# alguoo314/JASPER

Measured on AMD Instinct MI355X. Metric: assembly Mbp/s polished + Gk-mers/s counted, k=37, higher is better.
Workload: dtype u64

## Files before the change

include/jasper_hip.h:

```cpp
#ifndef JASPER_HIP_H
#define JASPER_HIP_H
#include <stddef.h>
#include <stdint.h>

#ifdef __cplusplus
extern "C" {
#endif

typedef struct jasper_table jasper_table;
typedef struct jasper_result jasper_result;

typedef struct jasper_fixrec {
    int64_t index;
    uint32_t chunk;
    uint32_t seqno;
    uint8_t pass;
    uint8_t kind;
    uint8_t newc;
    uint8_t oldc;
    uint32_t rep;
    uint32_t aux_off;
    uint32_t aux_len;
} jasper_fixrec;

#define JASPER_OK 0
#define JASPER_ERR -1
#define JASPER_ERR_CAPACITY -2
#define JASPER_ERR_FORMAT -3
#define JASPER_ERR_REFERENCE_EXIT -4

const char *jasper_last_error(void);
int jasper_device_count(int *n);
int jasper_request_cancel(int on);
int jasper_device_mem_info(int device, uint64_t *free_bytes, uint64_t *total_bytes);

int jasper_table_create(int k, uint64_t min_slots, int device, jasper_table **out);
int jasper_table_load_jf(const char *path, int device, jasper_table **out);
void jasper_table_destroy(jasper_table *t);
int jasper_table_load_jf_part(const char *path, int device, uint32_t part, uint32_t nparts, jasper_table **out);
int jasper_table_write_jf(jasper_table *t, const char *path, const char *const *cmdline, int n_cmdline);
int jasper_debug_mix(int k, int inverse, uint64_t hi, uint64_t lo, uint64_t out2[2]);
int jasper_table_info(jasper_table *t, int *k, uint64_t *slots, uint64_t *distinct, uint64_t *occurrences);
int jasper_table_sync(jasper_table *t);
int jasper_table_clear(jasper_table *t);

int jasper_count_bases(jasper_table *t, const char *bases, uint64_t n);
int jasper_count_bases_device(jasper_table *t, const void *d_bases, uint64_t n);
int jasper_count_reads_text(jasper_table *t, const char *text, uint64_t n);
int jasper_count_reads_files(jasper_table *t, const char *const *paths, int n_paths);
int jasper_count_reads_file_ranges(jasper_table *t, const char *const *paths, const int64_t *begins, const int64_t *ends, int n_paths);

int jasper_last_ingest(jasper_table *t, uint64_t *gpu_bytes, uint64_t *host_bytes);
int jasper_last_inflate(jasper_table *t, uint64_t stats[6]);
int jasper_histogram(jasper_table *t, uint64_t *out10002);
int jasper_histogram_part(jasper_table *t, uint32_t part, uint32_t nparts, uint64_t *out10002);
int jasper_histogram_is_fused(jasper_table *t);
int jasper_lookup(jasper_table *t, const char *chars, const int64_t *offsets, uint64_t n, uint32_t *out);

int jasper_table_export(jasper_table *t, uint64_t *n_entries, uint64_t *host_entries );
int jasper_table_import(jasper_table *t, const uint64_t *host_entries, uint64_t n_entries);
int jasper_table_export_device(jasper_table *t, uint64_t *n_entries, void **d_entries);
int jasper_table_import_device(jasper_table *t, const void *d_entries, uint64_t n_entries);
int jasper_table_export_to(jasper_table *t, void *d_dst, uint64_t cap_entries, uint64_t *n_entries);
int jasper_device_free(jasper_table *t, void *d_ptr);
int jasper_table_export_packed(jasper_table *t, void *d_dst, uint64_t cap_entries, uint64_t *n_entries, uint32_t part, uint32_t nparts);
int jasper_table_import_packed(jasper_table *t, const void *d_src, uint64_t n_entries, int mode);
int jasper_table_import_packed_multi(jasper_table *t, const void *const *d_srcs, const uint64_t *counts, uint32_t n_src);
int jasper_table_reserve(jasper_table *t, uint64_t min_slots);
int jasper_table_fit(jasper_table *t, double max_load);

int jasper_table_export_owner(jasper_table *t, void *d_dst, uint64_t cap_entries, uint32_t n_owners, uint64_t *counts);
int jasper_read_feed_start(jasper_table *t, const char *const *paths, const int64_t *begins, const int64_t *ends, int n_paths);
int jasper_read_feed_next(jasper_table *t, const void **d_bases, uint64_t *n);
int jasper_read_feed_release(jasper_table *t);
int jasper_count_exchange_plan(jasper_table *t, uint64_t piece_max, uint64_t records_max, uint32_t n_owners, uint64_t *out8);
int jasper_count_exchange_scan(jasper_table *t, const void *d_bases, uint64_t n, uint64_t pos, uint64_t end, uint64_t piece_max, uint32_t n_owners, void *d_deferred,
                               uint64_t deferred_cap, uint64_t *records);
int jasper_count_exchange_partition(jasper_table *t, uint64_t piece_max, uint64_t records_max, uint32_t n_owners, void *d_send, void *d_send_counts, void *d_deferred,
                                    uint64_t deferred_cap);
int jasper_count_exchange_dedupe(jasper_table *t, uint64_t piece_max, uint64_t records_max, uint32_t n_owners, void *d_send, void *d_send_counts, uint32_t *max_fill,
                                 int *count_bits);
int jasper_count_exchange_insert(jasper_table *t, const void *d_recv, const void *d_recv_counts, uint64_t piece_max, uint64_t records_max, uint32_t n_owners,
                                 uint32_t self, const void *d_deferred_all, uint64_t n_deferred_all, int whole_input, uint32_t slice_cap, int count_bits);
int jasper_table_export_file_ranges(jasper_table *t, void *d_dst, uint64_t cap_entries, uint32_t n_ranges, int size_log2, uint64_t *counts);
int jasper_table_write_jf_piece(jasper_table *t, const char *path, const char *const *cmdline, int n_cmdline, int size_log2, int what);
int jasper_table_ipc_handle(jasper_table *t, void *out64);
int jasper_table_attach_ipc(jasper_table *t, const void *handles, uint32_t n, uint32_t self);
int jasper_table_attach_tables(jasper_table *t, jasper_table *const *shards, uint32_t n, uint32_t self);
int jasper_table_detach(jasper_table *t);
int jasper_ipc_probe(int device, const void *handles, uint32_t n, uint32_t self);
uint32_t jasper_owner_of(uint64_t hash_lo, uint64_t hash_hi, uint32_t n);

int jasper_polish_batch(jasper_table *t, int n_chunks, const char *const *seqs, const int64_t *lens,
                        int solid_thre, int passes, int fix, jasper_result **out);
int jasper_polish_batch_device(jasper_table *t, int n_chunks, const void *d_text, const int64_t *offsets,
                               int solid_thre, int passes, int fix, jasper_result **out);
int jasper_result_num_chunks(const jasper_result *r);
int jasper_result_seq(const jasper_result *r, int chunk, const char **seq, int64_t *len);
int jasper_result_seq_len(const jasper_result *r, int chunk, int64_t *len);
int jasper_result_seq_device(const jasper_result *r, int chunk, const void **d_seq, int64_t *len);
int jasper_result_records(const jasper_result *r, const jasper_fixrec **recs, uint64_t *n);
int jasper_result_aux(const jasper_result *r, int chunk, const char **aux, uint64_t *n);
int jasper_result_qv(const jasper_result *r, int64_t out4[4]);
int jasper_result_qv_chunk(const jasper_result *r, int chunk, int64_t out4[4]);
int jasper_result_lookups(const jasper_result *r, uint64_t *n);
double jasper_result_seconds(const jasper_result *r);
int jasper_result_segments(const jasper_result *r, uint64_t *n_segments, uint64_t *n_respeculated);
int jasper_polish_cut_geometry(int k, int64_t out5[5]);
int jasper_result_retried(const jasper_result *r);
void jasper_result_free(jasper_result *r);

typedef struct jasper_report jasper_report;
typedef struct jasper_kmer_run { int64_t start; uint64_t n_kmers; uint64_t n_absent; uint32_t seq; uint32_t min_count; } jasper_kmer_run;
int jasper_kmer_report(jasper_table *t, int n_seqs, const char *const *seqs, const int64_t *lens, uint32_t thre, jasper_report **out);
int jasper_kmer_report_device(jasper_table *t, int n_seqs, const void *d_text, const int64_t *offsets, uint32_t thre, jasper_report **out);
int jasper_report_tile_windows(void);
int jasper_report_num_seqs(const jasper_report *r);
int jasper_report_counts(const jasper_report *r, int seq, uint64_t out4[4]);
int jasper_report_runs(const jasper_report *r, const jasper_kmer_run **runs, uint64_t *n);
double jasper_report_seconds(const jasper_report *r);
int jasper_report_retried(const jasper_report *r);
void jasper_report_free(jasper_report *r);

int jasper_spectrum_rows(void);
int jasper_table_spectrum(jasper_table *reads, jasper_table *assembly, uint64_t *out_cells , double *device_seconds);
// ... 227 lines not shown
```

jasper_amd/_lib.py:

```python
import ctypes as C
import os

_HERE = os.path.dirname(os.path.abspath(__file__))
LIB_PATH = os.environ.get("JASPER_AMD_LIB") or os.path.join(_HERE, "libjasper_hip.so")

JASPER_OK = 0
JASPER_ERR = -1
JASPER_ERR_CAPACITY = -2
JASPER_ERR_FORMAT = -3
JASPER_ERR_REFERENCE_EXIT = -4


class FixRec(C.Structure):
    _fields_ = [("index", C.c_int64), ("chunk", C.c_uint32), ("seqno", C.c_uint32), ("pass_", C.c_uint8),
                ("kind", C.c_uint8), ("newc", C.c_uint8), ("oldc", C.c_uint8), ("rep", C.c_uint32),
                ("aux_off", C.c_uint32), ("aux_len", C.c_uint32)]


assert C.sizeof(FixRec) == 32


class KmerRun(C.Structure):
    _fields_ = [("start", C.c_int64), ("n_kmers", C.c_uint64), ("n_absent", C.c_uint64), ("seq", C.c_uint32), ("min_count", C.c_uint32)]

# ... 22 lines not shown

assert C.sizeof(HapRun) == 24


class Variant(C.Structure):
    _fields_ = [("pos", C.c_int64), ("seq", C.c_uint32), ("ref_min", C.c_uint32), ("alt_min", C.c_uint32), ("ref", C.c_uint8), ("alt", C.c_uint8),
                ("kind", C.c_uint8), ("pad", C.c_uint8)]


assert C.sizeof(Variant) == 24


class Indel(C.Structure):
    _fields_ = [("pos", C.c_int64), ("seq", C.c_uint32), ("ref_min", C.c_uint32), ("alt_min", C.c_uint32), ("len", C.c_uint16), ("type", C.c_uint8),
                ("base", C.c_uint8), ("kind", C.c_uint8), ("pad", C.c_uint8 * 7)]


assert C.sizeof(Indel) == 32


class MixedIns(C.Structure):
    _fields_ = [("pos", C.c_int64), ("seq", C.c_uint32), ("ref_min", C.c_uint32), ("alt_min", C.c_uint32), ("bases", C.c_uint32), ("len", C.c_uint16),
                ("kind", C.c_uint8), ("pad", C.c_uint8 * 5)]


assert C.sizeof(MixedIns) == 32


class Compound(C.Structure):
    _fields_ = [("pos", C.c_int64), ("seq", C.c_uint32), ("ref_min", C.c_uint32), ("alt_min", C.c_uint32), ("ref_len", C.c_uint32), ("bases", C.c_uint64 * 2),
                ("len", C.c_uint16), ("pad", C.c_uint8 * 6)]


assert C.sizeof(Compound) == 48


class HetCluster(C.Structure):
    _fields_ = Compound._fields_


assert C.sizeof(HetCluster) == 48


class Edit(C.Structure):
    _fields_ = [("pos", C.c_int64), ("seq", C.c_uint32), ("ref_min", C.c_uint32), ("alt_min", C.c_uint32), ("ref_len", C.c_uint32), ("bases", C.c_uint64 * 2),
                ("len", C.c_uint16), ("source", C.c_uint8), ("round", C.c_uint8), ("pad", C.c_uint8 * 4)]


assert C.sizeof(Edit) == 48


class RepairRound(C.Structure):
    _fields_ = [("records", C.c_uint64), ("accepted", C.c_uint64), ("conflicts", C.c_uint64), ("ambiguous", C.c_uint64), ("unreliable_before", C.c_uint64),
                ("unreliable_after", C.c_uint64)]


assert C.sizeof(RepairRound) == 48


class GapSite(C.Structure):
    _fields_ = [("a", C.c_int64), ("q", C.c_int64), ("seq", C.c_uint32), ("ref_min", C.c_uint32), ("n_records", C.c_uint32), ("levels", C.c_uint32),
                ("trim_left", C.c_uint32), ("trim_right", C.c_uint32), ("kind", C.c_uint8), ("status", C.c_uint8), ("pad", C.c_uint8 * 6)]


assert C.sizeof(GapSite) == 48


class GapFill(C.Structure):
    _fields_ = [("pos", C.c_int64), ("bases_off", C.c_uint64), ("seq", C.c_uint32), ("ref_len", C.c_uint32), ("len", C.c_uint32), ("alt_min", C.c_uint32)]


assert C.sizeof(GapFill) == 32

_P = C.c_void_p
SYMBOLS = {
    "jasper_last_error": (C.c_char_p, []),
    "jasper_device_count": (C.c_int, [C.POINTER(C.c_int)]),
    "jasper_request_cancel": (C.c_int, [C.c_int]),
    "jasper_device_mem_info": (C.c_int, [C.c_int, C.POINTER(C.c_uint64), C.POINTER(C.c_uint64)]),
    "jasper_table_create": (C.c_int, [C.c_int, C.c_uint64, C.c_int, C.POINTER(_P)]),
    "jasper_table_load_jf": (C.c_int, [C.c_char_p, C.c_int, C.POINTER(_P)]),
    "jasper_table_destroy": (None, [_P]),
    "jasper_table_info": (C.c_int, [_P, C.POINTER(C.c_int), C.POINTER(C.c_uint64), C.POINTER(C.c_uint64), C.POINTER(C.c_uint64)]),
    "jasper_table_sync": (C.c_int, [_P]),
    "jasper_table_clear": (C.c_int, [_P]),
    "jasper_count_bases": (C.c_int, [_P, C.c_char_p, C.c_uint64]),
    "jasper_count_bases_device": (C.c_int, [_P, _P, C.c_uint64]),
    "jasper_count_reads_text": (C.c_int, [_P, C.c_char_p, C.c_uint64]),
    "jasper_count_reads_files": (C.c_int, [_P, C.POINTER(C.c_char_p), C.c_int]),
    "jasper_count_reads_file_ranges": (C.c_int, [_P, C.POINTER(C.c_char_p), C.POINTER(C.c_int64), C.POINTER(C.c_int64), C.c_int]),
    "jasper_table_load_jf_part": (C.c_int, [C.c_char_p, C.c_int, C.c_uint32, C.c_uint32, C.POINTER(_P)]),
    "jasper_table_write_jf": (C.c_int, [_P, C.c_char_p, C.POINTER(C.c_char_p), C.c_int]),
    "jasper_debug_mix": (C.c_int, [C.c_int, C.c_int, C.c_uint64, C.c_uint64, C.POINTER(C.c_uint64)]),
    "jasper_last_ingest": (C.c_int, [_P, C.POINTER(C.c_uint64), C.POINTER(C.c_uint64)]),
    "jasper_last_inflate": (C.c_int, [_P, C.POINTER(C.c_uint64)]),
    "jasper_histogram_part": (C.c_int, [_P, C.c_uint32, C.c_uint32, C.POINTER(C.c_uint64)]),
    "jasper_histogram_is_fused": (C.c_int, [_P]),
    "jasper_histogram": (C.c_int, [_P, C.POINTER(C.c_uint64)]),
    "jasper_lookup": (C.c_int, [_P, C.c_char_p, C.POINTER(C.c_int64), C.c_uint64, C.POINTER(C.c_uint32)]),
    "jasper_table_export": (C.c_int, [_P, C.POINTER(C.c_uint64), C.POINTER(C.c_uint64)]),
    "jasper_table_import": (C.c_int, [_P, C.POINTER(C.c_uint64), C.c_uint64]),
    "jasper_table_export_device": (C.c_int, [_P, C.POINTER(C.c_uint64), C.POINTER(_P)]),
    "jasper_table_import_device": (C.c_int, [_P, _P, C.c_uint64]),
    "jasper_table_export_to": (C.c_int, [_P, _P, C.c_uint64, C.POINTER(C.c_uint64)]),
    "jasper_device_free": (C.c_int, [_P, _P]),
    "jasper_table_export_packed": (C.c_int, [_P, _P, C.c_uint64, C.POINTER(C.c_uint64), C.c_uint32, C.c_uint32]),
    "jasper_table_import_packed": (C.c_int, [_P, _P, C.c_uint64, C.c_int]),
    "jasper_table_import_packed_multi": (C.c_int, [_P, C.POINTER(_P), C.POINTER(C.c_uint64), C.c_uint32]),
    "jasper_table_reserve": (C.c_int, [_P, C.c_uint64]),
    "jasper_table_fit": (C.c_int, [_P, C.c_double]),
    "jasper_read_feed_start": (C.c_int, [_P, C.POINTER(C.c_char_p), C.POINTER(C.c_int64), C.POINTER(C.c_int64), C.c_int]),
    "jasper_read_feed_next": (C.c_int, [_P, C.POINTER(C.c_void_p), C.POINTER(C.c_uint64)]),
    "jasper_read_feed_release": (C.c_int, [_P]),
    "jasper_count_exchange_plan": (C.c_int, [_P, C.c_uint64, C.c_uint64, C.c_uint32, C.POINTER(C.c_uint64)]),
    "jasper_count_exchange_scan": (C.c_int, [_P, _P, C.c_uint64, C.c_uint64, C.c_uint64, C.c_uint64, C.c_uint32, _P, C.c_uint64, C.POINTER(C.c_uint64)]),
    "jasper_count_exchange_partition": (C.c_int, [_P, C.c_uint64, C.c_uint64, C.c_uint32, _P, _P, _P, C.c_uint64]),
    "jasper_count_exchange_dedupe": (C.c_int, [_P, C.c_uint64, C.c_uint64, C.c_uint32, _P, _P, C.POINTER(C.c_uint32), C.POINTER(C.c_int)]),
    "jasper_count_exchange_insert": (C.c_int, [_P, _P, _P, C.c_uint64, C.c_uint64, C.c_uint32, C.c_uint32, _P, C.c_uint64, C.c_int, C.c_uint32, C.c_int]),
    "jasper_table_export_owner": (C.c_int, [_P, _P, C.c_uint64, C.c_uint32, C.POINTER(C.c_uint64)]),
    "jasper_table_export_file_ranges": (C.c_int, [_P, _P, C.c_uint64, C.c_uint32, C.c_int, C.POINTER(C.c_uint64)]),
    "jasper_table_write_jf_piece": (C.c_int, [_P, C.c_char_p, C.POINTER(C.c_char_p), C.c_int, C.c_int, C.c_int]),
    "jasper_table_ipc_handle": (C.c_int, [_P, _P]),
    "jasper_table_attach_ipc": (C.c_int, [_P, _P, C.c_uint32, C.c_uint32]),
    "jasper_table_attach_tables": (C.c_int, [_P, C.POINTER(_P), C.c_uint32, C.c_uint32]),
    "jasper_table_detach": (C.c_int, [_P]),
    "jasper_ipc_probe": (C.c_int, [C.c_int, _P, C.c_uint32, C.c_uint32]),
    "jasper_table_release_retired": (C.c_int, [_P]),
    "jasper_inflate_file": (C.c_int, [C.c_char_p, C.c_int, C.c_uint64, C.c_char_p, C.POINTER(C.c_uint64), C.POINTER(C.c_int)]),
    "jasper_inflate_file_device": (C.c_int, [C.c_int, C.c_char_p, C.c_uint64, C.c_char_p, C.POINTER(C.c_uint64), C.POINTER(C.c_uint64)]),
    "jasper_owner_of": (C.c_uint32, [C.c_uint64, C.c_uint64, C.c_uint32]),
    "jasper_polish_batch": (C.c_int, [_P, C.c_int, C.POINTER(C.c_char_p), C.POINTER(C.c_int64), C.c_int, C.c_int, C.c_int, C.POINTER(_P)]),
    "jasper_result_num_chunks": (C.c_int, [_P]),
    "jasper_polish_batch_device": (C.c_int, [_P, C.c_int, _P, C.POINTER(C.c_int64), C.c_int, C.c_int, C.c_int, C.POINTER(_P)]),
    "jasper_result_seq": (C.c_int, [_P, C.c_int, C.POINTER(_P), C.POINTER(C.c_int64)]),
    "jasper_result_seq_len": (C.c_int, [_P, C.c_int, C.POINTER(C.c_int64)]),
    "jasper_result_seq_device": (C.c_int, [_P, C.c_int, C.POINTER(_P), C.POINTER(C.c_int64)]),
    "jasper_result_records": (C.c_int, [_P, C.POINTER(C.POINTER(FixRec)), C.POINTER(C.c_uint64)]),
    "jasper_result_aux": (C.c_int, [_P, C.c_int, C.POINTER(_P), C.POINTER(C.c_uint64)]),
    "jasper_result_qv": (C.c_int, [_P, C.POINTER(C.c_int64)]),
    "jasper_result_qv_chunk": (C.c_int, [_P, C.c_int, C.POINTER(C.c_int64)]),
    "jasper_result_lookups": (C.c_int, [_P, C.POINTER(C.c_uint64)]),
    "jasper_result_seconds": (C.c_double, [_P]),
    "jasper_result_segments": (C.c_int, [_P, C.POINTER(C.c_uint64), C.POINTER(C.c_uint64)]),
    "jasper_polish_cut_geometry": (C.c_int, [C.c_int, C.POINTER(C.c_int64)]),
    "jasper_result_retried": (C.c_int, [_P]),
    "jasper_result_free": (None, [_P]),
    "jasper_kmer_report": (C.c_int, [_P, C.c_int, C.POINTER(C.c_char_p), C.POINTER(C.c_int64), C.c_uint32, C.POINTER(_P)]),
    "jasper_kmer_report_device": (C.c_int, [_P, C.c_int, _P, C.POINTER(C.c_int64), C.c_uint32, C.POINTER(_P)]),
    "jasper_report_tile_windows": (C.c_int, []),
    "jasper_report_num_seqs": (C.c_int, [_P]),
    "jasper_report_counts": (C.c_int, [_P, C.c_int, C.POINTER(C.c_uint64)]),
    "jasper_report_runs": (C.c_int, [_P, C.POINTER(C.POINTER(KmerRun)), C.POINTER(C.c_uint64)]),
    "jasper_report_seconds": (C.c_double, [_P]),
    "jasper_report_retried": (C.c_int, [_P]),
    "jasper_report_free": (None, [_P]),
    "jasper_spectrum_rows": (C.c_int, []),
    "jasper_table_spectrum": (C.c_int, [_P, _P, C.POINTER(C.c_uint64), C.POINTER(C.c_double)]),
    "jasper_copy_report": (C.c_int, [_P, _P, C.c_int, C.POINTER(C.c_char_p), C.POINTER(C.c_int64), C.c_uint32, C.c_uint32, C.POINTER(_P)]),
    "jasper_copy_report_device": (C.c_int, [_P, _P, C.c_int, _P, C.POINTER(C.c_int64), C.c_uint32, C.c_uint32, C.POINTER(_P)]),
    "jasper_copyrep_num_seqs": (C.c_int, [_P]),
    "jasper_copyrep_counts": (C.c_int, [_P, C.c_int, C.POINTER(C.c_uint64)]),
    "jasper_copyrep_runs": (C.c_int, [_P, C.POINTER(C.POINTER(CopyRun)), C.POINTER(C.c_uint64)]),
    "jasper_copyrep_seconds": (C.c_double, [_P]),
    "jasper_copyrep_retried": (C.c_int, [_P]),
    "jasper_copyrep_free": (None, [_P]),
    "jasper_dup_map": (C.c_int, [_P, _P, C.c_int, C.POINTER(C.c_char_p), C.POINTER(C.c_int64), C.c_uint32, C.c_uint32, C.POINTER(_P)]),
# ... 174 lines not shown
```

jasper_amd/csrc/capi.hip:

```cpp
#include "../../include/jasper_hip.h"
#include "ingest.hpp"
#include "polish_host.hpp"
#include "table.hpp"
#include "pgunzip.hpp"
#include "inflate_gpu.hpp"
#include "asmio.hpp"
#include "report.hpp"
#include "spectra.hpp"
#include "copies.hpp"
#include "hapmers.hpp"
#include "variants.hpp"
#include "indels.hpp"
#include "compound.hpp"
#include "repair.hpp"
#include "dups.hpp"
#include "gaps.hpp"
#include <zlib.h>
#include <algorithm>
#include <cmath>
#include <cstddef>
#include <cstring>
#include <string>
#include <vector>

// ... 134 lines not shown

int jasper_request_cancel(int on) { jk::g_cancel.store(on ? 1 : 0); return JASPER_OK; }

int jasper_device_mem_info(int device, uint64_t *free_bytes, uint64_t *total_bytes) {
    size_t f = 0, t = 0;
    hipError_t e = hipSetDevice(device);
    if (e == hipSuccess) e = hipMemGetInfo(&f, &t);
    if (e != hipSuccess) { g_err = std::string("hipMemGetInfo: ") + hipGetErrorString(e); return JASPER_ERR; }
    if (free_bytes) *free_bytes = (uint64_t)f;
    if (total_bytes) *total_bytes = (uint64_t)t;
    return JASPER_OK;
}

int jasper_table_create(int k, uint64_t min_slots, int device, jasper_table **out) {
    if (!out) { g_err = "null out"; return JASPER_ERR; }
    jasper_table *h = new jasper_table();
    int rc = h->t.init(k, min_slots, device, g_err);
    if (rc) { h->t.destroy(); delete h; return rc; }
    *out = h;
    return JASPER_OK;
}

int jasper_table_load_jf(const char *path, int device, jasper_table **out) {
    if (!out || !path) { g_err = "null argument"; return JASPER_ERR; }
    JfHeader h;
    int rc = jf_read_header(path, h, g_err);
    if (rc) return rc == -3 ? JASPER_ERR_FORMAT : JASPER_ERR;
    jasper_table *t = nullptr;
    rc = jasper_table_create(h.key_len / 2, std::max<uint64_t>(1u << 16, 2 * h.n_records), device, &t);
    if (rc) return rc;
    Table *T = &t->t;
    rc = T->load_jf_records(path, h.data_offset, h.n_records, h.key_len, h.counter_len, g_err);
    if (rc) { jasper_table_destroy(t); return rc < -1 ? rc : JASPER_ERR; }
    *out = t;
    return JASPER_OK;
}

int jasper_table_load_jf_part(const char *path, int device, uint32_t part, uint32_t nparts, jasper_table **out) {
    if (!out || !path || nparts == 0 || part >= nparts) { g_err = "bad argument"; return JASPER_ERR; }
    JfHeader h;
    int rc = jf_read_header(path, h, g_err);
    if (rc) return rc == -3 ? JASPER_ERR_FORMAT : JASPER_ERR;
    const uint64_t lo = h.n_records / nparts * part + std::min<uint64_t>(part, h.n_records % nparts);
    const uint64_t n = h.n_records / nparts + (part < h.n_records % nparts ? 1 : 0);
    const uint64_t rec = (uint64_t)((h.key_len + 7) / 8) + (uint64_t)h.counter_len;
    jasper_table *t = nullptr;
    rc = jasper_table_create(h.key_len / 2, std::max<uint64_t>(1u << 16, 2 * n), device, &t);
    if (rc) return rc;
    rc = t->t.load_jf_records(path, h.data_offset + lo * rec, n, h.key_len, h.counter_len, g_err);
    if (rc) { jasper_table_destroy(t); return rc < -1 ? rc : JASPER_ERR; }
    *out = t;
    return JASPER_OK;
}

int jasper_table_write_jf(jasper_table *t, const char *path, const char *const *cmdline, int n_cmdline) {
    if (!t || !path || n_cmdline < 0 || (n_cmdline && !cmdline)) { g_err = "null argument"; return JASPER_ERR; }
    return t->t.write_jf(path, cmdline, n_cmdline, g_err) ? JASPER_ERR : JASPER_OK;
}

int jasper_debug_mix(int k, int inverse, uint64_t hi, uint64_t lo, uint64_t out2[2]) {
    if (k < 1 || k > 64 || !out2) { g_err = "bad arguments"; return JASPER_ERR; }
    const u128 r = inverse ? unmix(mk(hi, lo), 2 * k) : mix(mk(hi, lo), 2 * k);
    out2[0] = r.hi;
    out2[1] = r.lo;
    return JASPER_OK;
}

void jasper_table_destroy(jasper_table *t) {
    if (!t) return;
    if (t->pending) (void)result_fetch(t->pending);
    t->t.destroy();
    delete t;
}

int jasper_table_info(jasper_table *t, int *k, uint64_t *slots, uint64_t *distinct, uint64_t *occurrences) {
    if (t->t.read_stats(g_err)) return JASPER_ERR;
    if (k) *k = t->t.k;
    if (slots) *slots = t->t.nslots;
    if (distinct) *distinct = t->t.h_stats[ST_DISTINCT];
    if (occurrences) *occurrences = t->t.h_stats[ST_OCCURRENCES];
    return JASPER_OK;
}

int jasper_table_sync(jasper_table *t) {
    CHK(hipSetDevice(t->t.device));
    CHK(jk_stream_wait(t->t.stream));
    return JASPER_OK;
}

int jasper_table_clear(jasper_table *t) { return t->t.clear(g_err) ? JASPER_ERR : JASPER_OK; }

int jasper_count_bases(jasper_table *t, const char *bases, uint64_t n) {
    t->t.reset_timing();
    return t->t.count_host(bases, n, g_err);
}

int jasper_count_bases_device(jasper_table *t, const void *d_bases, uint64_t n) {
    t->t.reset_timing();
    return t->t.count_device((const uint8_t *)d_bases, n, g_err);
}

int jasper_count_reads_text(jasper_table *t, const char *text, uint64_t n) {
    t->t.reset_timing();
    Table *T = &t->t;
    FastxParser p([T](const char *b, size_t m) { return T->count_host(b, m, g_err); });
    int rc = p.feed(text, n);
    if (!rc) rc = p.finish();
    if (rc && !p.error().empty()) g_err = p.error();
    return rc;
}

int jasper_count_reads_file_ranges(jasper_table *t, const char *const *paths, const int64_t *begins, const int64_t *ends, int n_paths) {
    if (!begins || !ends) { g_err = "null range arrays"; return JASPER_ERR; }
    t->t.reset_timing();
    Table *T = &t->t;
    T->ingest_gpu_bytes = T->ingest_host_bytes = 0;
    T->ingest_begin = begins;
    T->ingest_end = ends;
    const int rc = T->count_files_gpu(paths, n_paths, &T->ingest_gpu_bytes, &T->ingest_host_bytes, g_err);
    T->ingest_begin = T->ingest_end = nullptr;
    return rc < -1 ? rc : (rc ? JASPER_ERR : JASPER_OK);
}

int jasper_count_reads_files(jasper_table *t, const char *const *paths, int n_paths) {
    t->t.reset_timing();
    Table *T = &t->t;
    T->ingest_gpu_bytes = T->ingest_host_bytes = 0;
    for (uint64_t &v : T->inflate_stats) v = 0;
    if (!getenv("JASPER_INGEST_HOST")) {
        const int rc = T->count_files_gpu(paths, n_paths, &T->ingest_gpu_bytes, &T->ingest_host_bytes, g_err);
        return rc < -1 ? rc : (rc ? JASPER_ERR : JASPER_OK);
    }
    FastxParser p([T](const char *b, size_t m) { return T->count_host(b, m, g_err); });
    std::string e;
    int rc = parse_files(paths, n_paths, p, e);
    if (rc && !e.empty()) g_err = e;
    return rc;
}

int jasper_last_ingest(jasper_table *t, uint64_t *gpu_bytes, uint64_t *host_bytes) {
    if (gpu_bytes) *gpu_bytes = t->t.ingest_gpu_bytes;
    if (host_bytes) *host_bytes = t->t.ingest_host_bytes;
    return JASPER_OK;
}

int jasper_last_inflate(jasper_table *t, uint64_t stats[6]) {
    if (!t || !stats) { g_err = "bad argument"; return JASPER_ERR; }
    for (int i = 0; i < GZS_N; ++i) stats[i] = t->t.inflate_stats[i];
    return JASPER_OK;
}

int jasper_last_count_timing(jasper_table *t, double *kernel_ms, uint64_t *launches) {
    if (kernel_ms) *kernel_ms = t->t.count_kernel_ms;
    if (launches) *launches = t->t.count_launches;
    return JASPER_OK;
}

int jasper_last_count_stages(jasper_table *t, double stage_ms[8], uint64_t *partitioned_launches, int *path) {
    for (int i = 0; i < 8; ++i) stage_ms[i] = t->t.part_stage_ms[i];
    if (partitioned_launches) *partitioned_launches = t->t.count_partitioned_launches;
    if (path) *path = t->t.count_path;
    return JASPER_OK;
}

int jasper_histogram_part(jasper_table *t, uint32_t part, uint32_t nparts, uint64_t *out10002) {
    if (nparts == 0 || part >= nparts || !out10002) { g_err = "bad partition"; return JASPER_ERR; }
// ... 778 lines not shown
```

jasper_amd/csrc/polish_host.hip:

```cpp
#include "polish_host.hpp"
#include <algorithm>
#include <chrono>
#include <cstdio>
#include <cstdlib>
#include <cstring>
#include <thread>

namespace jk {

#define HIPCHK(x)                                                                     \
    do {                                                                              \
        hipError_t e_ = (x);                                                          \
        if (e_ != hipSuccess) {                                                       \
            err = std::string(#x) + ": " + hipGetErrorString(e_);                     \
            return -1;                                                                \
        }                                                                             \
    } while (0)

static inline size_t al256(size_t x) { return (x + 255) & ~(size_t)255; }

namespace {
struct DevBuf {
    void *p = nullptr;
    bool owned = false;
// ... 481 lines not shown
                pin_recs_used += nrec_pass;
                pin_aux_used += naux_pass;
            } else {
                HIPCHK(hipMemcpyAsync(&R.recs[r0], d_recs.p, nrec_pass * sizeof(FixRec), hipMemcpyDeviceToHost, st));
                if (naux_pass) HIPCHK(hipMemcpyAsync(aux_pass.back().data(), d_aux.p, naux_pass, hipMemcpyDeviceToHost, st));
                HIPCHK(jk_stream_wait(st));
            }
        }
        const bool carry = pass < passes;
        if (carry) HIPCHK(hipMemsetAsync(b_flags.p, 0, flag_items, st));
        launch_seg_stitch(b_segs.as<SegDev>(), (int)ns, (uint8_t *const *)dOut, carry ? (uint8_t *const *)ptrClsOut : nullptr,
                          carry ? (uint8_t *const *)ptrFlags : nullptr, st);
        HIPCHK(hipGetLastError());
        for (int c = 0; c < n_chunks; ++c) len[c] = newlen[c];
        if (!ordinary) HIPCHK(jk_stream_wait(st));
        std::swap(hIn, hOut);
        std::swap(dIn, dOut);
        if (pass == 0) { hOut = hSpare; dOut = dSpare; }
        std::swap(clsIn, clsOut);
        std::swap(ptrClsIn, ptrClsOut);
    }
    if (dbg) { (void)jk_stream_wait(st); fprintf(stderr, "[polish] passes: %.2f ms\n", now() - t_loop); }
    const double t_out = now();
    if (rc == 0) {
        HIPCHK(hipEventRecord(ev1, st));
        if (keep_on_device) {
            R.d_seqs.resize(n_chunks);
            R.d_lens.assign(len.begin(), len.end());
            for (int c = 0; c < n_chunks; ++c) R.d_seqs[c] = hIn[c];
        }
        bool packed_back = false;
        if (packed_io && !keep_on_device) {
            int64_t at = 0;
            for (int c = 0; c < n_chunks; ++c) { io_offs[c] = at; at += len[c]; }
            io_offs[n_chunks] = at;
            if ((size_t)at <= text_bytes && (size_t)at <= (size_t)total_len + (size_t)(RM * std::max<int64_t>(4096, total_len / 8)) + 64) {
                packed_back = true;
                HIPCHK(hipMemcpyAsync(b_iooffs.p, io_offs.data(), io_offs.size() * 8, hipMemcpyHostToDevice, st));
                launch_copy_chunks(dIn, b_pack.as<uint8_t>(), b_iooffs.as<int64_t>(), n_chunks, false, st);
                HIPCHK(hipGetLastError());
                if (at) HIPCHK(hipMemcpyAsync(io_stage, b_pack.p, (size_t)at, hipMemcpyDeviceToHost, st));
            }
        }
        for (int c = 0; c < n_chunks && !keep_on_device && !packed_back; ++c) {
            R.seqs[c].resize((size_t)len[c]);
            if (len[c]) HIPCHK(hipMemcpyAsync(&R.seqs[c][0], hIn[c], (size_t)len[c], hipMemcpyDeviceToHost, st));
        }
        HIPCHK(jk_stream_wait(st));
        if (packed_back)
            for (int c = 0; c < n_chunks; ++c) R.seqs[c].assign(reinterpret_cast<const char *>(io_stage) + io_offs[c], (size_t)len[c]);
        float ms = 0;
        HIPCHK(hipEventElapsedTime(&ms, ev0, ev1));
        R.seconds = ms * 1e-3;
        for (const PinnedPass &P : pinned_passes) {
            memcpy(&R.recs[P.r0], recs_p + P.rec_at, P.nrec * sizeof(FixRec));
            if (P.naux) memcpy(aux_pass[P.pass_i].data(), aux_p + P.aux_at, P.naux);
        }
        for (size_t p = 0; p < rec_pass_begin.size(); ++p) {
            const size_t b = rec_pass_begin[p], e = p + 1 < rec_pass_begin.size() ? rec_pass_begin[p + 1] : R.recs.size();
            for (size_t i = b; i < e; ++i) {
                FixRec &f = R.recs[i];
                if (f.kind == 'x') {
                    std::string &a = R.aux[f.chunk];
                    const size_t n = (size_t)f.aux_len + f.rep;
                    const uint32_t no = (uint32_t)a.size();
                    a.append(reinterpret_cast<const char *>(aux_pass[p].data()) + f.aux_off, n);
                    f.aux_off = no;
                }
            }
        }
        std::stable_sort(R.recs.begin(), R.recs.end(), [](const FixRec &a, const FixRec &b) {
            if (a.chunk != b.chunk) return a.chunk < b.chunk;
            if (a.pass != b.pass) return a.pass < b.pass;
            return a.seqno < b.seqno;
        });
    }
    (void)jk_stream_wait(st);
    if (dbg) fprintf(stderr, "[polish] D2H + record sort: %.2f ms; total %.2f ms\n", now() - t_out, now() - t_begin);
    (void)hipEventDestroy(ev0);
    (void)hipEventDestroy(ev1);
    return rc;
}

int run_polish(Table &T, int n_chunks, const char *const *seqs, const int64_t *lens, int solid_thre, int passes, int fix,
               PolishOut &R, std::string &err, bool device_in, bool keep_on_device, int roomy) {
    HIPCHK(hipSetDevice(T.device));
    if (T.materialize(err)) return -1;
    int lanes = T.polish_calls++ >= 1 && n_chunks >= 12 ? 3 : 1;
    if (const char *e = getenv("JASPER_POLISH_LANES")) lanes = atoi(e);
    if (getenv("JASPER_POLISH_DEBUG")) lanes = 1;
    lanes = std::max(1, std::min(std::min(lanes, (int)Table::POLISH_LANES_MAX), n_chunks / 2));
    if (lanes == 1) return run_polish_lane(T, 0, T.stream, n_chunks, seqs, lens, solid_thre, passes, fix, R, err, device_in, keep_on_device, roomy);

    std::vector<int> order(n_chunks);
    for (int c = 0; c < n_chunks; ++c) order[c] = c;
    std::stable_sort(order.begin(), order.end(), [&](int a, int b) { return lens[a] > lens[b]; });
    std::vector<std::vector<int>> mine(lanes);
    std::vector<int64_t> load(lanes, 0);
    for (int c : order) {
        int l = 0;
        for (int j = 1; j < lanes; ++j) if (load[j] < load[l]) l = j;
        mine[l].push_back(c);
        load[l] += lens[c];
    }
    for (auto &m : mine) std::sort(m.begin(), m.end());
    if (!T.polish_ev) HIPCHK(hipEventCreateWithFlags(&T.polish_ev, hipEventDisableTiming));
    HIPCHK(hipEventRecord(T.polish_ev, T.stream));
    for (int l = 1; l < lanes; ++l) {
        if (!T.polish_stream[l]) HIPCHK(hipStreamCreateWithFlags(&T.polish_stream[l], hipStreamNonBlocking));
        HIPCHK(hipStreamWaitEvent(T.polish_stream[l], T.polish_ev, 0));
    }
    std::vector<PolishOut> out(lanes);
    std::vector<std::string> errs(lanes);
    std::vector<int> rcs(lanes, 0);
    std::vector<std::vector<const char *>> lseqs(lanes);
    std::vector<std::vector<int64_t>> llens(lanes);
    for (int l = 0; l < lanes; ++l)
        for (int c : mine[l]) { lseqs[l].push_back(seqs[c]); llens[l].push_back(lens[c]); }
    auto run = [&](int l) {
        rcs[l] = run_polish_lane(T, l, l ? T.polish_stream[l] : T.stream, (int)mine[l].size(), lseqs[l].data(), llens[l].data(), solid_thre, passes, fix, out[l],
                                 errs[l], device_in, keep_on_device, roomy);
    };
    {
        std::vector<std::thread> th;
        for (int l = 1; l < lanes; ++l) th.emplace_back(run, l);
        run(0);
        for (auto &t : th) t.join();
    }
    for (int want : {-1, -4, -2})
        for (int l = 0; l < lanes; ++l)
            if (rcs[l] == want) { err = errs[l]; return want; }
    for (int l = 0; l < lanes; ++l)
        if (rcs[l]) { err = errs[l]; return rcs[l]; }
    R.seqs.assign(n_chunks, std::string());
    R.aux.assign(n_chunks, std::string());
    R.d_seqs.clear();
    R.d_lens.clear();
    if (keep_on_device) { R.d_seqs.assign(n_chunks, nullptr); R.d_lens.assign(n_chunks, 0); }
    R.recs.clear();
    R.qv[0] = R.qv[1] = R.qv[2] = R.qv[3] = 0;
    R.qv_chunk.assign((size_t)4 * n_chunks, 0);
    R.lookups = 0; R.seconds = 0; R.n_segments = 0; R.n_respeculated = 0;
    for (int l = 0; l < lanes; ++l) {
        PolishOut &O = out[l];
        for (size_t j = 0; j < mine[l].size(); ++j) {
            const int c = mine[l][j];
            R.seqs[c].swap(O.seqs[j]);
            R.aux[c].swap(O.aux[j]);
            if (keep_on_device) { R.d_seqs[c] = O.d_seqs[j]; R.d_lens[c] = O.d_lens[j]; }
            for (int q = 0; q < 4; ++q) R.qv_chunk[4 * (size_t)c + q] = O.qv_chunk[4 * j + q];
        }
        for (FixRec f : O.recs) { f.chunk = (uint32_t)mine[l][f.chunk]; R.recs.push_back(f); }
        for (int q = 0; q < 4; ++q) R.qv[q] += O.qv[q];
        R.lookups += O.lookups;
        R.n_segments += O.n_segments;
        R.n_respeculated += O.n_respeculated;
        R.seconds = std::max(R.seconds, O.seconds);
    }
    std::stable_sort(R.recs.begin(), R.recs.end(), [](const FixRec &a, const FixRec &b) {
        if (a.chunk != b.chunk) return a.chunk < b.chunk;
        if (a.pass != b.pass) return a.pass < b.pass;
        return a.seqno < b.seqno;
    });
    return 0;
}

}
```

jasper_amd/csrc/table.hpp:

```cpp
#pragma once
#include "kmer.hpp"
#include <atomic>
#include <functional>
#include <string>
#include <vector>

namespace jk {

extern std::atomic<int> g_cancel;


constexpr uint32_t MAX_SHARDS = 8;
struct TableDev {
    unsigned long long *slots;
    uint64_t mask;
    int s;
    int B;
    int k;
    unsigned long long *stats;
    unsigned long long *spill;
    uint64_t spill_cap;
    const unsigned long long *shard[MAX_SHARDS];
    uint32_t nshard;
    unsigned long long *ext;
// ... 204 lines not shown
    const Raw16 r = load16(text, pos, n);
    encode16(r.w, codes, inv);
}

template <typename Get>
__device__ __forceinline__ u128 encode_padded(int k, long n, Get get) {
    u128 m = mk(0, 0);
    int t = 0;
    const int lim = n < k ? (int)n : k;
    for (; t < lim; ++t) {
        int c = code(get(t));
        if (c < 0) break;
        m = bor(shl(m, 2), mk(0, (uint64_t)c));
    }
    if (t < k) m = shl(m, 2 * (k - t));
    return m;
}

struct PartGeom {
    int p1, p2, rbits;
    int recbits;
    uint32_t nblk1;
    uint32_t grid1;
    uint32_t nblk2;
    uint32_t cap1, cap2;
};

struct Table {
    int device = 0;
    int k = 0;
    hipStream_t stream = nullptr;
    TableDev d{};
    uint64_t nslots = 0;
    uint8_t *d_stage[2] = {nullptr, nullptr};
    uint8_t *h_stage[2] = {nullptr, nullptr};
    hipEvent_t ev_stage[2] = {nullptr, nullptr};
    size_t stage_bytes = 0;
    unsigned long long *h_stats = nullptr;
    double grow_at = 0.5;
    hipEvent_t ev_k0 = nullptr, ev_k1 = nullptr;
    double count_kernel_ms = 0;
    uint64_t count_launches = 0;
    void reset_timing() { count_kernel_ms = 0; count_launches = 0; count_partitioned_launches = 0; for (double &m : part_stage_ms) m = 0; }
    int launch_count(const uint8_t *d_piece, uint64_t len, uint64_t emit_from, std::string &err);
    bool partition_geometry(uint64_t piece_bases, PartGeom &G) const;
    int launch_count_partitioned(const uint8_t *d_piece, uint64_t len, uint64_t emit_from, const PartGeom &G, std::string &err);
    uint64_t count_partitioned_launches = 0;
    static constexpr int N_STAGES = 8;
    hipEvent_t ev_stage_t[N_STAGES + 1] = {};
    double part_stage_ms[N_STAGES] = {};
    int part_stage_n = 5;
    int count_path = 0;
    bool part_stage_pending = false;
    unsigned long long *part_defer_header = nullptr;
    bool part_slots_dirty_before = false, part_off = false;
    bool xchg_partitioned = false;
    bool xchg_deduped = false;
    static constexpr int HISTO_WORDS = 10002 + 6;
    unsigned long long *d_histo = nullptr;
    bool histo_cached = false, histo_request = false;
    double dup_ratio = 1.0;
    uint64_t size_hint = 0;
    struct WsBuf { void *p = nullptr; size_t bytes = 0; };
    static constexpr int POLISH_LANES_MAX = 4;
    static constexpr int WS_POLISH_MAX = 40, WS_COUNT = 40, WS_INGEST = 44, WS_XCHG = 51, WS_HOSTBASES = 55, WS_LANE0 = 56,
                         WS_GZ = WS_LANE0 + (POLISH_LANES_MAX - 1) * WS_POLISH_MAX,
                         WS_REPORT = WS_GZ + 5,
                         WS_SPECTRA = WS_REPORT + 8,
                         WS_COPIES = WS_SPECTRA + 1,
                         WS_VARIANTS = WS_COPIES + 8,
                         WS_INDELS = WS_VARIANTS + 8,
                         WS_MIXED = WS_INDELS + 4,
                         WS_COMPOUND = WS_MIXED + 2,
                         WS_CLUSTERS = WS_COMPOUND + 4,
                         WS_HAPMERS = WS_CLUSTERS + 2,
                         WS_REPAIR = WS_HAPMERS + 9,
                         WS_DUPS = WS_REPAIR + 4,
                         WS_GAPS = WS_DUPS + 9,
                         WS_SLOTS = WS_GAPS + 14;
    WsBuf ws[WS_SLOTS];
    hipStream_t polish_stream[POLISH_LANES_MAX] = {nullptr, nullptr, nullptr, nullptr};
    hipEvent_t polish_ev = nullptr;
    uint64_t polish_calls = 0;
    hipStream_t jf_stream = nullptr;
    hipStream_t ingest_stream = nullptr;
    hipStream_t ingest_copy_stream = nullptr;
    hipEvent_t ingest_copy_ev[2] = {nullptr, nullptr};
    void *workspace(int id, size_t bytes, std::string &err);
    void wait_streams();
    static constexpr int PIN_PER_LANE = 8, PIN_SLOTS = PIN_PER_LANE * POLISH_LANES_MAX;
    WsBuf pin[PIN_SLOTS];
    void *pinned(int id, size_t bytes, std::string &err);

    static int min_log2_slots(int k);
    int init(int k, uint64_t min_slots, int device, std::string &err);
    void destroy();
    int read_stats(std::string &err);
    int zero_slots(unsigned long long *slots, uint64_t n, std::string &err);
    bool slots_dirty = false;
    int materialize(std::string &err) { if (!slots_dirty) return 0; slots_dirty = false; return zero_slots(d.slots, nslots, err); }
    int clear(std::string &err);
    int ensure_capacity(uint64_t upcoming_kmers, std::string &err);
    int grow(int new_s, std::string &err);
    int resize(int new_s, std::string &err);
    int ensure_narrow(std::string &err);
    int fit(double max_load, std::string &err);
    int after_batch(std::string &err);
    int count_device(const uint8_t *d_bases, uint64_t n, std::string &err, uint64_t first_new = 0);
    int count_host(const char *bases, uint64_t n, std::string &err);
    int count_files_gpu(const char *const *paths, int n_paths, uint64_t *gpu_bytes, uint64_t *host_bytes, std::string &err);
    uint64_t ingest_gpu_bytes = 0, ingest_host_bytes = 0;
    uint64_t inflate_stats[6] = {};
    hipStream_t gz_stream = nullptr;
    const int64_t *ingest_begin = nullptr, *ingest_end = nullptr;
    std::function<int(const uint8_t *d_bases, uint64_t n)> bases_sink;
    struct Feed;
    Feed *feed = nullptr;
    int feed_start(const char *const *paths, const int64_t *begins, const int64_t *ends, int n_paths, std::string &err);
    int feed_next(const void **d_bases, uint64_t *n, std::string &err);
    int feed_release(std::string &err);
    void feed_stop();
    char *h_ingest = nullptr;
    size_t ingest_chunk = 0;
    int histogram(uint64_t *out10002, std::string &err);
    int histogram_part(uint32_t part, uint32_t nparts, uint64_t *out10002, std::string &err);
    void part_span(uint32_t part, uint32_t nparts, uint64_t &first, uint64_t &span) const;
    int lookup_strings(const char *chars, const int64_t *offsets, uint64_t n, uint32_t *out, std::string &err);
    int export_entries(uint64_t *n_out, unsigned long long **d_entries_out, std::string &err);
    int import_entries(const unsigned long long *d_entries, uint64_t n, std::string &err);
    int export_packed(void *d_dst, uint64_t cap, uint64_t *n_out, uint32_t part, uint32_t nparts, std::string &err);
    int import_packed(const void *d_src, uint64_t n, int mode, std::string &err);
    int packed_count_refused(std::string &err);
    int import_packed_multi(const void *const *d_srcs, const uint64_t *counts, uint32_t n_src, std::string &err);
    int reserve(uint64_t min_slots, std::string &err);
    int export_owner(void *d_dst, uint64_t cap, uint32_t nown, int sort_r, uint64_t *counts_out, std::string &err);
    int xchg_plan(uint64_t piece_max, uint64_t records_max, uint32_t nown, uint64_t out[8], std::string &err);
    int xchg_scan(const uint8_t *d_bases, uint64_t n, uint64_t pos, uint64_t end, uint64_t piece_max, uint32_t nown, void *d_defer, uint64_t defer_cap, uint64_t *records,
                  std::string &err);
    int xchg_partition(uint64_t piece_max, uint64_t records_max, uint32_t nown, void *d_send, void *d_send_cnt, void *d_defer, uint64_t defer_cap, std::string &err);
    int xchg_dedupe(uint64_t piece_max, uint64_t records_max, uint32_t nown, void *d_send, void *d_send_cnt, uint32_t *max_fill, int *cbits_out, std::string &err);
    int xchg_insert(const void *d_recv, const void *d_recv_cnt, uint64_t piece_max, uint64_t records_max, uint32_t nown, uint32_t self, const void *d_defer_all,
                    uint64_t n_defer_all, int whole_input, uint32_t slice_cap, int cbits, std::string &err);
    int ipc_handle(void *out64, std::string &err);
    int attach_ipc(const void *handles64, uint32_t n, uint32_t self, std::string &err);
    int attach_tables(Table *const *peers, uint32_t n, uint32_t self, std::string &err);
    void detach_shards();
    bool exported = false;
    std::vector<void *> retired;
    void release_retired();
    void *ipc_mapped[MAX_SHARDS] = {};
    int write_jf(const char *path, const char *const *cmdline, int n_cmd, std::string &err, int r_bits = -1, int what = 0);
    int load_jf_records(const char *path, uint64_t data_offset, uint64_t n_records, int key_len_bits, int counter_len, std::string &err);
};

}
```

jasper_amd/table.py:

```python
import ctypes as C

from . import _lib
from ._lib import FixRec, check


class PolishResult:

    def __init__(self, lib, handle, n_chunks, want_str, raw_records, aux, qv, lookups, seconds):
        self._L = lib
        self._h = handle
        self._n = n_chunks
        self._want_str = want_str
        self._seqs = None
        self._raw = raw_records
        self._records = None
        self.aux = aux
        self.qv = qv
        self.lookups = lookups
        self.seconds = seconds
        self.segments = 0
        self.respeculated = 0
        self.retried = False

    def __del__(self):
# ... 464 lines not shown

    def count_file_ranges(self, ranges):
        n = len(ranges)
        arr = (C.c_char_p * max(n, 1))(*[r[0].encode() for r in ranges])
        b = (C.c_int64 * max(n, 1))(*[int(r[1]) for r in ranges])
        e = (C.c_int64 * max(n, 1))(*[int(r[2]) for r in ranges])
        check(self._L.jasper_count_reads_file_ranges(self._h, arr, b, e, n))

    def feed_start(self, ranges):
        n = len(ranges)
        arr = (C.c_char_p * max(n, 1))(*[r[0].encode() for r in ranges])
        b = (C.c_int64 * max(n, 1))(*[int(r[1]) for r in ranges])
        e = (C.c_int64 * max(n, 1))(*[int(r[2]) for r in ranges])
        check(self._L.jasper_read_feed_start(self._h, arr, b, e, n))

    def feed_next(self):
        p, n = C.c_void_p(0), C.c_uint64(0)
        check(self._L.jasper_read_feed_next(self._h, C.byref(p), C.byref(n)))
        return (p.value or 0), n.value

    def feed_release(self):
        check(self._L.jasper_read_feed_release(self._h))

    def last_ingest(self):
        a, b = C.c_uint64(0), C.c_uint64(0)
        check(self._L.jasper_last_ingest(self._h, C.byref(a), C.byref(b)))
        return a.value, b.value

    INFLATE_KEYS = ("decoders", "accepted", "device_bytes", "host_bytes", "slabs", "members")

    def last_inflate(self):
        st = (C.c_uint64 * 6)()
        check(self._L.jasper_last_inflate(self._h, st))
        return dict(zip(self.INFLATE_KEYS, (int(v) for v in st)))

    def count_text(self, text):
        if isinstance(text, str):
            text = text.encode()
        check(self._L.jasper_count_reads_text(self._h, text, len(text)))

    def count_bases(self, bases):
        if isinstance(bases, str):
            bases = bases.encode()
        check(self._L.jasper_count_bases(self._h, bases, len(bases)))

    def count_bases_device(self, dev_ptr, n):
        check(self._L.jasper_count_bases_device(self._h, C.c_void_p(dev_ptr), int(n)))

    def count_timing(self):
        ms = C.c_double(0)
        n = C.c_uint64(0)
        check(self._L.jasper_last_count_timing(self._h, C.byref(ms), C.byref(n)))
        return ms.value, n.value

    STAGE_NAMES = {1: ("part1_kernel", "part2_kernel", "region_insert_kernel", "deferred_import3h_kernel"),
                   3: ("part1_kernel", "part2_by_owner_kernel", "region_insert_kernel", "(unused)", "deferred_import3h_kernels"),
                   0: ()}

    def count_stages(self):
        ms = (C.c_double * 8)()
        n = C.c_uint64(0)
        path = C.c_int(0)
        check(self._L.jasper_last_count_stages(self._h, ms, C.byref(n), C.byref(path)))
        self._count_path = path.value
        return list(ms)[:len(self.STAGE_NAMES.get(path.value, ()))] or list(ms)[:5], n.value

    def count_path(self):
        self.count_stages()
        return self._count_path

    def clear(self):
        check(self._L.jasper_table_clear(self._h))

    def sync(self):
        check(self._L.jasper_table_sync(self._h))

    def info(self):
        k = C.c_int(0)
        slots = C.c_uint64(0)
        distinct = C.c_uint64(0)
        occ = C.c_uint64(0)
        check(self._L.jasper_table_info(self._h, C.byref(k), C.byref(slots), C.byref(distinct), C.byref(occ)))
        return dict(k=k.value, slots=slots.value, distinct=distinct.value, occurrences=occ.value)

    def histogram_is_fused(self):
        return bool(self._L.jasper_histogram_is_fused(self._h))

    def histogram(self):
        out = (C.c_uint64 * 10002)()
        check(self._L.jasper_histogram(self._h, out))
        return list(out)

    def histogram_part(self, part, nparts):
        out = (C.c_uint64 * 10002)()
        check(self._L.jasper_histogram_part(self._h, int(part), int(nparts), out))
        return list(out)

    def histo_rows(self):
        import numpy as np
        out = (C.c_uint64 * 10002)()
        check(self._L.jasper_histogram(self._h, out))
        h = np.frombuffer(out, dtype=np.uint64)
        nz = np.flatnonzero(h[1:]) + 1
        return list(zip(nz.tolist(), h[nz].tolist()))

    def lookup(self, strings):
        n = len(strings)
        if n == 0:
            return []
        bs = [s.encode() if isinstance(s, str) else bytes(s) for s in strings]
        offs = (C.c_int64 * (n + 1))()
        tot = 0
        for i, b in enumerate(bs):
            offs[i] = tot
            tot += len(b)
        offs[n] = tot
        out = (C.c_uint32 * n)()
        check(self._L.jasper_lookup(self._h, b"".join(bs), offs, n, out))
        return list(out)

    def export_entries(self):
        import numpy as np
        n = C.c_uint64(0)
        check(self._L.jasper_table_export(self._h, C.byref(n), None))
        arr = np.zeros((max(int(n.value), 1), 3), dtype=np.uint64)
        cap = C.c_uint64(arr.shape[0])
        check(self._L.jasper_table_export(self._h, C.byref(cap), arr.ctypes.data_as(C.POINTER(C.c_uint64))))
        return arr[: int(cap.value)]

    def import_entries(self, arr):
        import numpy as np
        arr = np.ascontiguousarray(arr, dtype=np.uint64)
        if arr.size == 0:
            return
        check(self._L.jasper_table_import(self._h, arr.ctypes.data_as(C.POINTER(C.c_uint64)), arr.shape[0]))

    def export_device(self):
        n = C.c_uint64(0)
        p = C.c_void_p()
        check(self._L.jasper_table_export_device(self._h, C.byref(n), C.byref(p)))
        return p.value, int(n.value)

    def export_to(self, dev_ptr, cap_entries):
        n = C.c_uint64(0)
        check(self._L.jasper_table_export_to(self._h, C.c_void_p(dev_ptr), int(cap_entries), C.byref(n)))
        return int(n.value)

    def export_packed(self, dev_ptr, cap_entries, part=0, nparts=1):
        n = C.c_uint64(0)
        check(self._L.jasper_table_export_packed(self._h, C.c_void_p(dev_ptr), int(cap_entries), C.byref(n), int(part), int(nparts)))
        return int(n.value)

    def import_packed(self, dev_ptr, n, mode=0):
        check(self._L.jasper_table_import_packed(self._h, C.c_void_p(dev_ptr), int(n), int(mode)))

    def import_packed_multi(self, dev_ptrs, counts):
        n = len(dev_ptrs)
        ps = (C.c_void_p * n)(*[int(p) for p in dev_ptrs])
        cs = (C.c_uint64 * n)(*[int(c) for c in counts])
        check(self._L.jasper_table_import_packed_multi(self._h, ps, cs, n))

    def reserve(self, min_slots):
        check(self._L.jasper_table_reserve(self._h, int(min_slots)))

    def fit(self, max_load=0.5):
        check(self._L.jasper_table_fit(self._h, float(max_load)))
# ... 471 lines not shown
```

Baseline: 3037.

## Probe stream concurrency before using multiple polish lanes

Before the first multi-lane polish, the code creates candidate streams at varying priorities and runs paired sleep kernels to check whether two streams actually execute concurrently. Only streams that pass are kept as polish lanes, and the lane count is capped at the number of concurrent streams unless overridden by environment. This aims to avoid splitting polish work across streams that serialize on the device, at the cost of a one-time probing delay and extra stream creation. It also adds an introspection API reporting lane decisions.

```diff
diff --git a/include/jasper_hip.h b/include/jasper_hip.h
--- a/include/jasper_hip.h
+++ b/include/jasper_hip.h
@@ -41,6 +41,7 @@
 int jasper_table_write_jf(jasper_table *t, const char *path, const char *const *cmdline, int n_cmdline);
 int jasper_debug_mix(int k, int inverse, uint64_t hi, uint64_t lo, uint64_t out2[2]);
 int jasper_table_info(jasper_table *t, int *k, uint64_t *slots, uint64_t *distinct, uint64_t *occurrences);
+int jasper_polish_lane_info(jasper_table *t, int64_t out[6]);
 int jasper_table_sync(jasper_table *t);
 int jasper_table_clear(jasper_table *t);
 
diff --git a/jasper_amd/_lib.py b/jasper_amd/_lib.py
--- a/jasper_amd/_lib.py
+++ b/jasper_amd/_lib.py
@@ -128,6 +128,7 @@
     "jasper_table_load_jf": (C.c_int, [C.c_char_p, C.c_int, C.POINTER(_P)]),
     "jasper_table_destroy": (None, [_P]),
     "jasper_table_info": (C.c_int, [_P, C.POINTER(C.c_int), C.POINTER(C.c_uint64), C.POINTER(C.c_uint64), C.POINTER(C.c_uint64)]),
+    "jasper_polish_lane_info": (C.c_int, [_P, C.POINTER(C.c_int64)]),
     "jasper_table_sync": (C.c_int, [_P]),
     "jasper_table_clear": (C.c_int, [_P]),
     "jasper_count_bases": (C.c_int, [_P, C.c_char_p, C.c_uint64]),
diff --git a/jasper_amd/csrc/capi.hip b/jasper_amd/csrc/capi.hip
--- a/jasper_amd/csrc/capi.hip
+++ b/jasper_amd/csrc/capi.hip
@@ -240,6 +240,20 @@
     return JASPER_OK;
 }
 
+int jasper_polish_lane_info(jasper_table *t, int64_t out[6]) {
+    if (!t || !out) { g_err = "bad arguments"; return JASPER_ERR; }
+    const Table &T = t->t;
+    int64_t streams = 1;
+    for (int l = 1; l < Table::POLISH_LANES_MAX; ++l) streams += T.polish_stream[l] != nullptr;
+    out[0] = T.polish_lanes_last;
+    out[1] = T.polish_lanes_concurrent;
+    out[2] = T.polish_stream_choices;
+    out[3] = streams;
+    out[4] = T.polish_stream_candidates;
+    out[5] = (int64_t)(T.polish_probe_us * 1e3f);
+    return JASPER_OK;
+}
+
 int jasper_table_sync(jasper_table *t) {
     CHK(hipSetDevice(t->t.device));
     CHK(jk_stream_wait(t->t.stream));
diff --git a/jasper_amd/csrc/polish_host.hip b/jasper_amd/csrc/polish_host.hip
--- a/jasper_amd/csrc/polish_host.hip
+++ b/jasper_amd/csrc/polish_host.hip
@@ -587,14 +587,84 @@
     return rc;
 }
 
+__global__ void lane_delay_kernel(int trips) {
+    for (int i = 0; i < trips; ++i) __builtin_amdgcn_s_sleep(127);
+}
+
+namespace {
+constexpr int LANE_DELAY_TRIPS = 24;
+constexpr int LANE_PROBE_REPS = 5;
+constexpr int LANE_CANDIDATES = 6;
+}
+
+static int lanes_concurrent(hipStream_t a, hipStream_t b, hipEvent_t (&ev)[3], bool &yes, float &one_us, std::string &err) {
+    int votes = 0;
+    hipLaunchKernelGGL(lane_delay_kernel, dim3(1), dim3(64), 0, b, 1);
+    HIPCHK(hipGetLastError());
+    HIPCHK(jk_stream_wait(b));
+    for (int rep = 0; rep < LANE_PROBE_REPS; ++rep) {
+        float one = 0, ta = 0, tb = 0;
+        HIPCHK(hipEventRecord(ev[0], a));
+        hipLaunchKernelGGL(lane_delay_kernel, dim3(1), dim3(64), 0, a, LANE_DELAY_TRIPS);
+        HIPCHK(hipEventRecord(ev[1], a));
+        HIPCHK(jk_stream_wait(a));
+        HIPCHK(hipEventElapsedTime(&one, ev[0], ev[1]));
+        HIPCHK(hipEventRecord(ev[0], a));
+        hipLaunchKernelGGL(lane_delay_kernel, dim3(1), dim3(64), 0, a, LANE_DELAY_TRIPS);
+        hipLaunchKernelGGL(lane_delay_kernel, dim3(1), dim3(64), 0, b, LANE_DELAY_TRIPS);
+        HIPCHK(hipEventRecord(ev[1], a));
+        HIPCHK(hipEventRecord(ev[2], b));
+        HIPCHK(hipGetLastError());
+        HIPCHK(jk_stream_wait(a));
+        HIPCHK(jk_stream_wait(b));
+        HIPCHK(hipEventElapsedTime(&ta, ev[0], ev[1]));
+        HIPCHK(hipEventElapsedTime(&tb, ev[0], ev[2]));
+        if (std::max(ta, tb) < 1.5f * one) ++votes;
+        one_us = one * 1e3f;
+    }
+    yes = 2 * votes > LANE_PROBE_REPS;
+    if (getenv("JASPER_TEST_LANES_SERIAL")) yes = false;
+    return 0;
+}
+
+static int choose_lane_streams(Table &T, std::string &err) {
+    ++T.polish_stream_choices;
+    HIPCHK(jk_stream_wait(T.stream));
+    hipEvent_t ev[3] = {nullptr, nullptr, nullptr};
+    for (hipEvent_t &e : ev) HIPCHK(hipEventCreate(&e));
+    int lo = 0, hi = 0;
+    HIPCHK(hipDeviceGetStreamPriorityRange(&lo, &hi));
+    std::vector<hipStream_t> rejected;
+    int have = 1, rc = 0;
+    for (int c = 0; c < LANE_CANDIDATES && have < 3 && rc == 0; ++c) {
+        hipStream_t s = nullptr;
+        if (hipStreamCreateWithPriority(&s, hipStreamNonBlocking, c < 2 ? 0 : c < 4 ? hi : lo) != hipSuccess) { err = "polish: hipStreamCreateWithPriority"; rc = -1; break; }
+        ++T.polish_stream_candidates;
+        bool ok = true;
+        for (int l = 0; l < have && ok && rc == 0; ++l)
+            rc = lanes_concurrent(l ? T.polish_stream[l] : T.stream, s, ev, ok, T.polish_probe_us, err);
+        if (rc == 0 && ok) T.polish_stream[have++] = s;
+        else rejected.push_back(s);
+    }
+    for (hipStream_t s : rejected) { (void)jk_stream_wait(s); (void)hipStreamDestroy(s); }
+    for (hipEvent_t e : ev) (void)hipEventDestroy(e);
+    if (rc) return rc;
+    T.polish_lanes_concurrent = have;
+    return 0;
+}
+
 int run_polish(Table &T, int n_chunks, const char *const *seqs, const int64_t *lens, int solid_thre, int passes, int fix,
                PolishOut &R, std::string &err, bool device_in, bool keep_on_device, int roomy) {
     HIPCHK(hipSetDevice(T.device));
     if (T.materialize(err)) return -1;
     int lanes = T.polish_calls++ >= 1 && n_chunks >= 12 ? 3 : 1;
-    if (const char *e = getenv("JASPER_POLISH_LANES")) lanes = atoi(e);
+    const char *const lanes_env = getenv("JASPER_POLISH_LANES");
+    if (lanes_env) lanes = atoi(lanes_env);
     if (getenv("JASPER_POLISH_DEBUG")) lanes = 1;
     lanes = std::max(1, std::min(std::min(lanes, (int)Table::POLISH_LANES_MAX), n_chunks / 2));
+    if (lanes > 1 && !T.polish_lanes_concurrent && choose_lane_streams(T, err)) return -1;
+    if (lanes > 1 && !lanes_env) lanes = std::min(lanes, T.polish_lanes_concurrent);
+    T.polish_lanes_last = lanes;
     if (lanes == 1) return run_polish_lane(T, 0, T.stream, n_chunks, seqs, lens, solid_thre, passes, fix, R, err, device_in, keep_on_device, roomy);
 
     std::vector<int> order(n_chunks);
diff --git a/jasper_amd/csrc/table.hpp b/jasper_amd/csrc/table.hpp
--- a/jasper_amd/csrc/table.hpp
+++ b/jasper_amd/csrc/table.hpp
@@ -310,6 +310,11 @@
     hipStream_t polish_stream[POLISH_LANES_MAX] = {nullptr, nullptr, nullptr, nullptr};
     hipEvent_t polish_ev = nullptr;
     uint64_t polish_calls = 0;
+    int polish_lanes_concurrent = 0;
+    int polish_lanes_last = 0;
+    uint32_t polish_stream_choices = 0;
+    uint32_t polish_stream_candidates = 0;
+    float polish_probe_us = 0;
     hipStream_t jf_stream = nullptr;
     hipStream_t ingest_stream = nullptr;
     hipStream_t ingest_copy_stream = nullptr;
diff --git a/jasper_amd/table.py b/jasper_amd/table.py
--- a/jasper_amd/table.py
+++ b/jasper_amd/table.py
@@ -570,6 +570,11 @@
         occ = C.c_uint64(0)
         check(self._L.jasper_table_info(self._h, C.byref(k), C.byref(slots), C.byref(distinct), C.byref(occ)))
         return dict(k=k.value, slots=slots.value, distinct=distinct.value, occurrences=occ.value)
+
+    def polish_lanes(self):
+        out = (C.c_int64 * 6)()
+        check(self._L.jasper_polish_lane_info(self._h, out))
+        return dict(lanes=out[0], concurrent=out[1], passed=out[1] >= 3, choices=out[2], streams=out[3], candidates=out[4], probe_us=out[5] / 1e3)
 
     def histogram_is_fused(self):
         return bool(self._L.jasper_histogram_is_fused(self._h))
```

After: 3029, median of 2. No clear change (-0.3%).
